# ymxlzgy/commonscenes

Hardware: AMD Instinct MI355X
Metric: DDIM denoise steps/sec (32 objects, 16^3 latent) (higher is better)
Workload: dtype f32 (operands as fp16 hi+lo pairs, fp32 accumulate)

## Files before the change

commonscenes_amd/csrc/cs_epilogue.h:

```cpp
#pragma once
#include "cs_common.h"

typedef unsigned cs_u32x4 __attribute__((ext_vector_type(4)));

template <class D, class M>
__device__ __forceinline__ f32x4 cs_epi_terms4(const D& d, f32x4 v, M m, int n) {
  if (d.bias) v += *reinterpret_cast<const f32x4*>(d.bias + n);
  if (d.scale) v = v * *reinterpret_cast<const f32x4*>(d.scale + n) + *reinterpret_cast<const f32x4*>(d.shift + n);
  if (d.rowvec) v += *reinterpret_cast<const f32x4*>(d.rowvec + (int64_t)(m / d.rv_rows) * d.ldrv + n);
  if (d.act != CS_ACT_NONE) {
#pragma unroll
    for (int e = 0; e < 4; ++e) v[e] = cs_act(v[e], d.act);
  }
  if (d.res) v += *reinterpret_cast<const f32x4*>(d.res + (int64_t)m * d.ldr + n);
  return v;
}
template <class D>
__device__ __forceinline__ float cs_epi_terms1(const D& d, float v, float bias, float scale, float shift, int m, int n) {
  v += bias;
  if (d.scale) v = v * scale + shift;
  if (d.rowvec) v += d.rowvec[(int64_t)(m / d.rv_rows) * d.ldrv + n];
  v = cs_act(v, d.act);
  if (d.res) v += d.res[(int64_t)m * d.ldr + n];
  return v;
}

__device__ __forceinline__ f32x4 cs_geglu4(f32x4 x, const f32x4& g) {
#pragma unroll
  for (int e = 0; e < 4; ++e) x[e] = x[e] * cs_gelu(g[e]);
  return x;
}

__device__ __forceinline__ cs_u32x4 cs_pair16(const f32x4& v, float out_scale, bool odd, float& oamax) {
  typedef _Float16 h4 __attribute__((ext_vector_type(4)));
  typedef unsigned u32x2 __attribute__((ext_vector_type(2)));
  h4 hi, lo;
#pragma unroll
  for (int e = 0; e < 4; ++e) {
    const float o = v[e] * out_scale;
    oamax = fmaxf(oamax, fabsf(o));
    hi[e] = (_Float16)o;
    lo[e] = (_Float16)(o - (float)hi[e]);
  }
  const u32x2 H = __builtin_bit_cast(u32x2, hi), L = __builtin_bit_cast(u32x2, lo);
  const u32x2 send = odd ? H : L;
  u32x2 recv;
  recv[0] = (unsigned)__builtin_amdgcn_update_dpp(0, (int)send[0], 0xB1, 0xF, 0xF, true);
  recv[1] = (unsigned)__builtin_amdgcn_update_dpp(0, (int)send[1], 0xB1, 0xF, 0xF, true);
  cs_u32x4 r;
  r[0] = odd ? recv[0] : H[0];
  r[1] = odd ? recv[1] : H[1];
  r[2] = odd ? L[0] : recv[0];
  r[3] = odd ? L[1] : recv[1];
  return r;
}
__device__ __forceinline__ int cs_pair_off(int col) { return (col >> 4) * 64 + ((col & 8) ? 32 : 0) + ((col & 4) ? 16 : 0); }
template <class D>
__device__ __forceinline__ void cs_pair_flag(const D& d, bool opair, float oamax) {
  if (opair && d.status && oamax >= 65504.f) atomicOr(d.status, CS_STATUS_F16X3_OVERFLOW);
}

__device__ __forceinline__ void cs_colsum_lanes16(double (*sc)[64], const double (&x)[4], int rl, int cl, double (&tot)[4]) {
  __syncthreads();
#pragma unroll
  for (int e = 0; e < 4; ++e) sc[rl][cl * 4 + e] = x[e];
  __syncthreads();
  if (rl == 0) {
#pragma unroll
    for (int e = 0; e < 4; ++e) {
      double t = 0.0;
      for (int r2 = 0; r2 < 16; ++r2) t += sc[r2][cl * 4 + e];
      tot[e] = t;
    }
  }
}
template <class D>
__device__ __forceinline__ void cs_colsum_staged(const D& d, const float* col, int ld, int rows, int tile, int n) {
  double ts = 0.0, tq = 0.0;
  for (int r2 = 0; r2 < rows; ++r2) {
    const double x = (double)col[r2 * ld];
    ts += x;
    tq += x * x;
  }
  double* o = d.gn_part + ((int64_t)tile * d.gn_ld + n) * 2;
  o[0] = ts;
  o[1] = tq;
}
```

commonscenes_amd/csrc/cs_gemm_f16x3.hip:

```cpp
#include <cstdlib>
#include <cstring>
#include "cs_f16x3.h"
#include "cs_epilogue.h"
#include <type_traits>
#include <utility>

namespace {

using cs16::h8;
using cs16::split8;
using cs16::wait_vmcnt;
using cs16::BKH;
using cs16::A_SCALE_DEFAULT;
using cs16::OOB;
constexpr int MAX_TAPS = 27;
#ifndef CS_ABLATE
#define CS_ABLATE 0
#endif

struct CsClsBatch {
  const void* w[8];
  const void* w_lo[8];
  float acc_scale[8];
  int n;
};

template <int NT, int BM, int BN>
__device__ __forceinline__ void fused_splitk_reduce(const CsFuseK& f, const float* __restrict__ ws, unsigned char* smem, int M,
                                                    int cout, int m0, int n0, int splits, int otile, int tid) {
  typedef unsigned u32x4 __attribute__((ext_vector_type(4)));
  typedef unsigned u32x2 __attribute__((ext_vector_type(2)));
  typedef _Float16 h4 __attribute__((ext_vector_type(4)));
  int32_t* const arrive = f.sync + 2 * otile;
  asm volatile("s_waitcnt vmcnt(0)" ::: "memory");
  __syncthreads();
  int* const tick = reinterpret_cast<int*>(smem);
  if (tid == 0) *tick = __hip_atomic_fetch_add(arrive, 1, __ATOMIC_RELAXED, __HIP_MEMORY_SCOPE_AGENT);
  __syncthreads();
  const int R = f.reducers;
  const int split = *tick - (splits - R);
  if (split < 0) return;
  if (tid == 0) {
    int spins = 0;
    while (__hip_atomic_load(arrive, __ATOMIC_RELAXED, __HIP_MEMORY_SCOPE_AGENT) < splits) {
      __builtin_amdgcn_s_sleep(4);
      if (++spins > (1 << 23)) {
        if (f.status) atomicOr(f.status, CS_STATUS_SPLITK_TIMEOUT);
        break;
      }
    }
  }
  __syncthreads();
  constexpr int C4 = BN / 4;
  constexpr int UNITS = 16 * C4;
  static_assert(UNITS % 2 == 0 && BN <= NT && 16 * BN * 4 <= 32768, "fused split-K reduce geometry");
  float* const lv = reinterpret_cast<float*>(smem);
  const __amdgpu_buffer_rsrc_t wrs = __builtin_amdgcn_make_buffer_rsrc(
      (void*)ws, 0, (unsigned)((int64_t)splits * M * cout * 4), 0x00020000);
  const bool gstat = f.gn_part != nullptr, opair = f.out_format == 2;
  const int rows_per = BM / R;
  float oamax = 0.f;
  for (int blk = 0; blk < rows_per / 16; ++blk) {
    const int r0 = split * rows_per + 16 * blk;
    if (m0 + r0 >= M) break;
    for (int u0 = 0; u0 < UNITS; u0 += NT) {
      const int u = u0 + tid;
      const int lrow = u / C4, c4 = u - lrow * C4;
      const int m = m0 + r0 + lrow, n = n0 + 4 * c4;
      const bool ok = u < UNITS && m < M && n < cout;
      f32x4 v = {0.f, 0.f, 0.f, 0.f};
      if (ok) {
        const unsigned off0 = (unsigned)(((int64_t)m * cout + n) * 4);
        const unsigned sstride = (unsigned)((int64_t)M * cout * 4);
        v = __builtin_bit_cast(f32x4, __builtin_amdgcn_raw_buffer_load_b128(wrs, off0, 0, 16));
        for (int s = 1; s < splits; s += 8) {
          f32x4 t[8];
#pragma unroll
          for (int q = 0; q < 8; ++q)
            if (s + q < splits)
              t[q] = __builtin_bit_cast(f32x4, __builtin_amdgcn_raw_buffer_load_b128(wrs, off0 + (unsigned)(s + q) * sstride, 0, 16));
#pragma unroll
          for (int q = 0; q < 8; ++q)
            if (s + q < splits) v += t[q];
        }
        v = cs_epi_terms4(f, v, m, n);
      }
      if (gstat && u < UNITS) *reinterpret_cast<f32x4*>(lv + lrow * BN + 4 * c4) = v;
      if (opair) {
        h4 hi, lo;
#pragma unroll
        for (int e = 0; e < 4; ++e) {
          const float o = v[e] * f.out_scale;
          oamax = fmaxf(oamax, fabsf(o));
          hi[e] = (_Float16)o;
          lo[e] = (_Float16)(o - (float)hi[e]);
        }
        const u32x2 H = __builtin_bit_cast(u32x2, hi), L = __builtin_bit_cast(u32x2, lo);
        const bool odd = tid & 1;
        const u32x2 send = odd ? H : L;
        u32x2 recv;
        recv[0] = (unsigned)__builtin_amdgcn_update_dpp(0, (int)send[0], 0xB1, 0xF, 0xF, true);
        recv[1] = (unsigned)__builtin_amdgcn_update_dpp(0, (int)send[1], 0xB1, 0xF, 0xF, true);
        u32x4 r;
        r[0] = odd ? recv[0] : H[0];
        r[1] = odd ? recv[1] : H[1];
        r[2] = odd ? L[0] : recv[0];
        r[3] = odd ? L[1] : recv[1];
        if (ok) {
          char* row = reinterpret_cast<char*>(f.out + (int64_t)m * f.ldo);
          *reinterpret_cast<u32x4*>(row + (n >> 4) * 64 + ((n & 8) ? 32 : 0) + ((n & 4) ? 16 : 0)) = r;
        }
      } else if (ok) {
        *reinterpret_cast<f32x4*>(f.out + (int64_t)m * f.ldo + n) = v;
      }
    }
    if (gstat) {
      __syncthreads();
      if (tid < BN && n0 + tid < cout) {
        double ts = 0.0, tq = 0.0;
#pragma unroll
        for (int r2 = 0; r2 < 16; ++r2) {
          const double d = (double)lv[r2 * BN + tid];
          ts += d;
          tq += d * d;
        }
        double* o = f.gn_part + ((int64_t)((m0 + r0) / 16) * f.gn_ld + n0 + tid) * 2;
        o[0] = ts;
        o[1] = tq;
      }
      __syncthreads();
    }
  }
  cs_pair_flag(f, opair, oamax);
  __syncthreads();
  if (tid == 0) {
    const int d = __hip_atomic_fetch_add(arrive + 1, 1, __ATOMIC_RELAXED, __HIP_MEMORY_SCOPE_AGENT);
    if (d == R - 1) {
      __hip_atomic_store(arrive, 0, __ATOMIC_RELAXED, __HIP_MEMORY_SCOPE_AGENT);
      __hip_atomic_store(arrive + 1, 0, __ATOMIC_RELAXED, __HIP_MEMORY_SCOPE_AGENT);
    }
  }
}

template <class F, int... I>
__device__ __forceinline__ void static_steps(std::integer_sequence<int, I...>, F&& f) {
  (f(std::integral_constant<int, I>{}), ...);
}

template <int WMB, int WNB, int WAVES_M, int WAVES_N, bool PRE, int SLAB = 0, bool PAIR = false, int TPK = 9, bool PW = false>
__global__ __launch_bounds__(64 * WAVES_M * WAVES_N, 2) void conv_gemm_f16x3_kernel(const CsConvGemm p, int M, int tiles_n,
                                                              int taps_hw, int kw_, int kg_per_tap,
                                                              long long x_bytes, unsigned w_bytes, int vec_epilogue,
                                                              int splits, int omap_f, int omap_p_in, const CsClsBatch cb,
                                                              const CsFuseK fz, int u_base, int u_count) {
  constexpr int BM = 32 * WMB * WAVES_M;
  constexpr int BN = 32 * WNB * WAVES_N;
  constexpr int NW = WAVES_M * WAVES_N;
  constexpr int NT = 64 * NW;
  static_assert(!SLAB || (WMB <= 2 && WAVES_N == 1), "slab path: one or two row blocks per wave");
  static_assert(!PAIR || (!PRE && SLAB == 0), "interleaved operand pairs: per-tap gather path only");
  static_assert(TPK == 9 || ((TPK == 4 || TPK == 3) && SLAB != 0), "taps per kd: 3x3 or (slab path only) 2x2 / 3x1");
  static_assert(!PW || SLAB == 0, "pointwise GEMMs take the gather path (there is one tap)");
  constexpr int KW_ = TPK == 9 ? 3 : TPK == 4 ? 2 : 1;
  constexpr int KH_ = TPK / KW_;
  constexpr int SLAB_ROWS = BM + (KH_ - 1) * SLAB + (KW_ - 1);
  constexpr int SLAB_IMG_WI = (SLAB_ROWS + 31) / 32;
  constexpr int SLAB_WI = PRE ? 2 * SLAB_IMG_WI : (SLAB_ROWS + 15) / 16;
  constexpr int SLAB_IMG = SLAB_IMG_WI * 1024;
  constexpr int SLAB_BYTES = SLAB ? SLAB_WI * 1024 : 0;
  constexpr int RING0 = 2 * SLAB_BYTES;
  constexpr int A_BYTES = SLAB ? 0 : BM * 64;
  constexpr int B_BYTES = 2 * BN * 16;
  constexpr int STAGE = A_BYTES + 2 * B_BYTES;
#ifdef CS_RING3
  constexpr int NSTAGE = 3;
#else
#ifdef CS_PW_RING3
  constexpr int NSTAGE = (BM == 64 && BN == 64) ? 6 : (TPK == 4 ? 4 : 3);
#else
#ifndef CS_RING64
#define CS_RING64 6
#endif
  constexpr int NSTAGE = (BM == 64 && BN == 64) ? CS_RING64 : ((TPK == 4 || (PW && BM == 256 && BN == 224)) ? 4 : 3);
#endif
#endif
  constexpr int PF = NSTAGE - 1;
  constexpr int DUMP = RING0 + NSTAGE * STAGE;
  constexpr int ROWBASE = DUMP + 1024;
  constexpr int DELTA = ROWBASE + (SLAB ? 0 : BM * 4);
  constexpr int ROWMIN = DELTA + (SLAB ? 0 : MAX_TAPS * BM * 2);
  constexpr int EP_KU = (4 * (32 * WNB / 4) + 63) / 64;
  constexpr int EPI_NEED = NW * (16 * 32 * WNB) + NW * 2 * EP_KU * 1024 + 2048;
  constexpr int OTAB = ((ROWMIN + 16 > EPI_NEED) ? ROWMIN + 16 : EPI_NEED);
  constexpr int LDS_BYTES = OTAB + (TPK == 4 ? BM * 4 : 0);
  constexpr short INVALID = (short)0x8000;
  constexpr int A_WI = BM / 16;
  constexpr int B_WI = BN / 32;
  constexpr int A_PW = SLAB ? 0 : A_WI / NW;
  constexpr int A_PWN = A_PW > 0 ? A_PW : 1;
  constexpr int B_PW = (2 * B_WI + NW - 1) / NW;
  constexpr int D = A_PW + B_PW;
  static_assert(A_WI % NW == 0, "A tile must split evenly over the waves");
  static_assert(D <= 7, "vmcnt immediates");
  __shared__ __attribute__((aligned(16))) unsigned char smem[LDS_BYTES];

  const int tid = threadIdx.x;
  const int lane = tid & 63;
  const int wave = __builtin_amdgcn_readfirstlane(tid >> 6);
  const int l31 = lane & 31;
  const int half = lane >> 5;
  const int wm0 = (wave / WAVES_N) * (32 * WMB);
  const int wn0 = (wave % WAVES_N) * (32 * WNB);

  int tile;
  {
    const int nblk = gridDim.x, b = blockIdx.x;
    const int q = nblk >> 3, r = nblk & 7, xcd = b & 7, within = b >> 3;
    tile = (xcd < r ? xcd * (q + 1) : r * (q + 1) + (xcd - r) * q) + within;
  }
  const void* w_hi_ = p.w;
  const void* w_lo_ = p.w_lo;
  float acc_scale_ = p.acc_scale;
  int pad_d = p.pd, pad_h = p.ph, pad_w = p.pw, omap_p = omap_p_in;
  int cls_id = 0;
  if constexpr (TPK == 4) {
    if (cb.n > 1) {
      const int per_cls = ((M + BM - 1) / BM) * tiles_n * splits;
      const int cls = tile / per_cls;
      cls_id = cls;
      tile -= cls * per_cls;
      w_hi_ = cb.w[cls];
      w_lo_ = cb.w_lo[cls];
      acc_scale_ = cb.acc_scale[cls];
      const int nw = 1 + (omap_f & 1), nh = 1 + ((omap_f >> 1) & 1);
      const int qw = cls % nw, qh = (cls / nw) % nh, qd = cls / (nw * nh);
      pad_d = (omap_f & 4) ? 1 - qd : 1;
      pad_h = (omap_f & 2) ? 1 - qh : 1;
      pad_w = (omap_f & 1) ? 1 - qw : 1;
      omap_p = (qd << 2) | (qh << 1) | qw;
    }
  }
  int split, tn, tm;
  if (TPK == 3 && u_count > 0) {
    const int R = ((M + BM - 1) / BM) / (omap_p_in > 1 ? omap_p_in : 1);
    const int r = tile % R;
    tile /= R;
    split = tile % splits;
    const int u = u_base + tile / splits;
    tn = u % tiles_n;
    tm = (u / tiles_n) * R + r;
  } else if (SLAB != 0 && splits > 1) {
    const int tiles_m = (M + BM - 1) / BM;
    tm = tile % tiles_m;
    tile /= tiles_m;
    split = tile % splits;
    tn = tile / splits;
  } else {
    split = tile % splits;
    tile /= splits;
    tn = tile % tiles_n;
    tm = tile / tiles_n;
  }
  const int m0 = tm * BM;
  const int n0 = tn * BN;
  if constexpr (TPK == 3) {
    if (omap_p_in > 1) {
      const int tiles_m = (M + BM - 1) / BM;
      const int q = tm / (tiles_m / omap_p_in);
      w_hi_ = reinterpret_cast<const char*>(p.w) + (size_t)q * w_bytes;
      w_lo_ = reinterpret_cast<const char*>(p.w_lo) + (size_t)q * w_bytes;
    }
  }

  const __amdgpu_buffer_rsrc_t hrs = __builtin_amdgcn_make_buffer_rsrc((void*)w_hi_, 0, w_bytes, 0x00020000);
  const __amdgpu_buffer_rsrc_t lrs = __builtin_amdgcn_make_buffer_rsrc((void*)w_lo_, 0, w_bytes, 0x00020000);

  const int ntaps = p.kd * taps_hw;
  int* rowbase = reinterpret_cast<int*>(smem + ROWBASE);
  int* rowmin = reinterpret_cast<int*>(smem + ROWMIN);
  short* delta = reinterpret_cast<short*>(smem + DELTA);
  if constexpr (!SLAB && !PW) {
  if (tid == 0) *rowmin = 0x7fffffff;
  __syncthreads();
  {
    const int vdin = p.din << p.ud, vhin = p.hin << p.uh, vwin = p.win << p.uw;
    constexpr int TPR = NT / BM >= 1 ? NT / BM : 1;
    for (int row = tid / TPR; row < BM; row += NT / TPR) {
      const int sub = tid % TPR;
      const int m = m0 + row;
      int mm = m < M ? m : 0;
      const int ow = mm % p.wout;
      mm /= p.wout;
      const int oh = mm % p.hout;
      mm /= p.hout;
      const int od = mm % p.dout;
      const int n = mm / p.dout;
      const int cd = min(max(od * p.sd - pad_d, 0), vdin - 1) >> p.ud;
      const int ch = min(max(oh * p.sh - pad_h, 0), vhin - 1) >> p.uh;
      const int cw = min(max(ow * p.sw - pad_w, 0), vwin - 1) >> p.uw;
      const int base = ((n * p.din + cd) * p.hin + ch) * p.win + cw;
      if (sub == 0) {
        rowbase[row] = base;
        if (m < M) atomicMin(rowmin, base);
      }
      const int vd0 = od * p.sd - pad_d, vh0 = oh * p.sh - pad_h, vw0 = ow * p.sw - pad_w;
      int t = 0;
      for (int kd_ = 0; kd_ < p.kd; ++kd_)
        for (int kh_ = 0; kh_ < p.kh; ++kh_)
          for (int kwi = 0; kwi < kw_; ++kwi, ++t) {
            if (t % TPR != sub) continue;
            short dl = INVALID;
            const int vd = vd0 + kd_, vh = vh0 + kh_, vw = vw0 + kwi;
            if (m < M && (unsigned)vd < (unsigned)vdin && (unsigned)vh < (unsigned)vhin &&
                (unsigned)vw < (unsigned)vwin) {
              const int r = ((n * p.din + (vd >> p.ud)) * p.hin + (vh >> p.uh)) * p.win + (vw >> p.uw);
              dl = (short)(r - base);
            }
            delta[t * BM + row] = dl;
          }
    }
  }
  __syncthreads();
  }

  const int row_lo = SLAB ? max(0, m0 - pad_d * p.hin * p.win - pad_h * p.win - pad_w)
                     : PW ? m0 : __builtin_amdgcn_readfirstlane(*rowmin);
  const long long x_skip = (long long)row_lo * p.lda * (PRE ? 2 : 4);
  const long long x_left = x_bytes - x_skip;
  const unsigned x_win = x_left > 0xFFE00000LL ? 0xFFE00000u : (unsigned)x_left;
  const __amdgpu_buffer_rsrc_t xrs =
      __builtin_amdgcn_make_buffer_rsrc((void*)((const char*)p.x + x_skip), 0, x_win, 0x00020000);
  const __amdgpu_buffer_rsrc_t xlrs = __builtin_amdgcn_make_buffer_rsrc(
      (void*)((const char*)(PRE ? p.x_lo : (const void*)p.x) + x_skip), 0, x_win, 0x00020000);

  float a_scale = p.a_scale;
  if constexpr (!PRE && !PAIR) {
    if (p.a_bound) {
      const float m = *p.a_bound;
      int ex = 0;
      float s2 = 1.0995116e12f;
      if (m > 0.f && m < 3.0e38f) {
        (void)frexpf(65000.0f / m, &ex);
        s2 = ldexpf(1.0f, min(max(ex - 1, -8), 40));
      }
      acc_scale_ *= a_scale / s2;
      a_scale = s2;
    }
  }
  const int chunks_per_tap = kg_per_tap >> 1;
  const int nk_all = ntaps * chunks_per_tap;
  constexpr int KGRAN = SLAB ? TPK : 1;
  const int per_split = ((nk_all / KGRAN + splits - 1) / splits) * KGRAN;
  const int k_first = split * per_split;
#if CS_ABLATE & 2048
  const int nk = 0;
#else
  const int nk = max(0, min(nk_all, k_first + per_split) - k_first);
#endif

  int a_rowbase[A_PWN];
  unsigned a_piece[A_PWN];
  int a_rowidx[A_PWN];
#pragma unroll
  for (int i = 0; i < A_PW; ++i) {
    const int w = wave * A_PW + i;
    if constexpr (PRE) {
      const int within = w % (A_WI / 2);
      const int row = 32 * within + (lane >> 1);
      a_rowidx[i] = row;
      if constexpr (PW) a_rowbase[i] = (m0 + row < M) ? row : -1;
      else a_rowbase[i] = rowbase[row] - row_lo;
      a_piece[i] = (unsigned)(((lane & 1) ^ ((row >> 3) & 1)) * 8);
    } else {
      const int row = 16 * w + (lane >> 2);
      a_rowidx[i] = row;
      if constexpr (PW) a_rowbase[i] = (m0 + row < M) ? row : -1;
      else a_rowbase[i] = rowbase[row] - row_lo;
      a_piece[i] = (unsigned)(((lane & 3) ^ ((row >> 2) & 3)) * 4);
    }
  }
  unsigned b_off[B_PW];
#pragma unroll
  for (int i = 0; i < B_PW; ++i) {
    const int v = wave * B_PW + i;
    const int img = v / B_WI;
    const int u = (v - img * B_WI) * 64 + lane;
    const int kg = u / BN;
    const int n = u - kg * BN;
    b_off[i] = (v < 2 * B_WI && n0 + n < p.cout) ? (unsigned)((kg * p.cout + n0 + n) * 16) : OOB;
  }

  auto issue_dma = [&](int tap, int cc, int stage) {
    unsigned char* st = smem + RING0 + stage * STAGE;
    const bool skip_a = ((CS_ABLATE & 128) && tap % 3 != 0) || ((CS_ABLATE & 256) && tap % 9 != 0);
#pragma unroll
    for (int i = 0; i < A_PW; ++i) {
      if (skip_a) break;
      const int c = cc * BKH + (int)a_piece[i];
      constexpr unsigned ESZ = PRE ? 2u : 4u;
      unsigned off;
      if constexpr (PW) {
        off = (a_rowbase[i] >= 0 && c < p.cin) ? (unsigned)a_rowbase[i] * ((unsigned)p.lda * ESZ) + (unsigned)c * ESZ : OOB;
      } else {
        const short dl = delta[tap * BM + a_rowidx[i]];
        off = (dl != INVALID && c < p.cin)
                  ? (unsigned)(a_rowbase[i] + (int)dl) * ((unsigned)p.lda * ESZ) + (unsigned)c * ESZ
                  : OOB;
      }
      if (CS_ABLATE & 2) off = OOB;
      if ((CS_ABLATE & 64) && off != OOB) off &= 0x3FF0u;
      const int w = wave * A_PW + i;
      if constexpr (PRE) {
        if (w >= A_WI / 2)
          __builtin_amdgcn_raw_ptr_buffer_load_lds(xlrs, st + w * 1024, 16, off, 0, 0, 0);
        else
          __builtin_amdgcn_raw_ptr_buffer_load_lds(xrs, st + w * 1024, 16, off, 0, 0, 0);
      } else {
        __builtin_amdgcn_raw_ptr_buffer_load_lds(xrs, st + w * 1024, 16, off, 0, 0, 0);
      }
    }
    const unsigned kbase = (unsigned)((tap * kg_per_tap + cc * 2) * p.cout) * 16u;
#pragma unroll
    for (int i = 0; i < B_PW; ++i) {
      const int v = wave * B_PW + i;
      const int img = v / B_WI;
      unsigned off = (b_off[i] == OOB || cc >= chunks_per_tap) ? OOB : b_off[i] + kbase;
      if (CS_ABLATE & 2) off = OOB;
      if ((CS_ABLATE & 64) && off != OOB) off &= 0x3FF0u;
      unsigned char* dst = (v < 2 * B_WI) ? st + A_BYTES + img * B_BYTES + (v - img * B_WI) * 1024 : smem + DUMP;
      if (img == 1)
        __builtin_amdgcn_raw_ptr_buffer_load_lds(lrs, dst, 16, off, 0, 0, 0);
      else
        __builtin_amdgcn_raw_ptr_buffer_load_lds(hrs, dst, 16, off, 0, 0, 0);
    }
  };

  f32x16 acc[WMB][WNB];
#pragma unroll
  for (int i = 0; i < WMB; ++i)
#pragma unroll
    for (int j = 0; j < WNB; ++j)
#pragma unroll
      for (int r = 0; r < 16; ++r) acc[i][j][r] = 0.f;

  int dtap = k_first % ntaps, dcc = k_first / ntaps;
  auto advance = [&]() {
    if (++dtap == ntaps) {
      dtap = 0;
      ++dcc;
    }
  };
#pragma unroll
  for (int q = 0; q < PF; ++q) {
    issue_dma(dtap, dcc, q);
    advance();
  }

  int a_frag[WMB][2];
#pragma unroll
  for (int i = 0; i < WMB; ++i) {
    const int row = wm0 + 32 * i + l31;
    if constexpr (PRE) {
      a_frag[i][0] = row * 32 + ((half ^ ((row >> 3) & 1)) * 16);
      a_frag[i][1] = a_frag[i][0] + BM * 32;
    } else {
      const int s = (row >> 2) & 3;
      a_frag[i][0] = row * 64 + (((2 * half) ^ s) * 16);
      a_frag[i][1] = row * 64 + (((2 * half + 1) ^ s) * 16);
    }
  }
  const int b_frag = A_BYTES + (half * BN + wn0 + l31) * 16;

  float amax = 0.f;
  auto load_a = [&](int st, h8 (&hi)[WMB], h8 (&lo)[WMB]) {
    const unsigned char* s = smem + RING0 + st * STAGE;
#pragma unroll
    for (int i = 0; i < WMB; ++i) {
      if constexpr (PRE) {
        hi[i] = *reinterpret_cast<const h8*>(s + a_frag[i][0]);
        lo[i] = *reinterpret_cast<const h8*>(s + a_frag[i][1]);
      } else {
        const f32x4 x0 = *reinterpret_cast<const f32x4*>(s + a_frag[i][0]);
        const f32x4 x1 = *reinterpret_cast<const f32x4*>(s + a_frag[i][1]);
#if CS_ABLATE & 512
        hi[i] = __builtin_bit_cast(h8, x0);
        lo[i] = __builtin_bit_cast(h8, x1);
#else
        if constexpr (PAIR) {
          hi[i] = __builtin_bit_cast(h8, x0);
          lo[i] = __builtin_bit_cast(h8, x1);
        } else {
          split8(x0, x1, a_scale, hi[i], lo[i], amax);
        }
#endif
      }
    }
  };
  constexpr int SLAB_PW = (SLAB_WI + NW - 1) / NW;
  const int s_w = p.win, s_hw = p.hin * p.win;
  const int s_rows = p.nb * p.din * s_hw;
  const int s_need = BM + (KH_ - 1) * s_w + (KW_ - 1);
  unsigned vmask[WMB];
  int sl_row[SLAB_PW];
  unsigned sl_piece[SLAB_PW];
  int sl_a0[WMB][TPK];
  if constexpr (SLAB != 0) {
#pragma unroll
    for (int i = 0; i < WMB; ++i) {
      const int rowl = wm0 + 32 * i + l31;
#pragma unroll
      for (int t9 = 0; t9 < TPK; ++t9) {
        const int prow = rowl + (t9 / KW_) * s_w + t9 % KW_;
        if constexpr (PRE)
          sl_a0[i][t9] = prow * 32 + (((half ^ (prow >> 3)) & 1) << 4);
        else
          sl_a0[i][t9] = prow * 64 + ((((2 * half) ^ (prow >> 2)) & 3) << 4);
      }
      vmask[i] = 0;
      const int m = m0 + rowl;
      if (m < M) {
        int mm = m;
        const int ow = mm % p.win;
        mm /= p.win;
        const int oh = mm % p.hin;
        mm /= p.hin;
        const int od = mm % p.din;
#pragma unroll
        for (int t = 0; t < 3 * TPK; ++t) {
          const int kd_ = t / TPK, kh_ = (t % TPK) / KW_, kwi = t % KW_;
          if ((unsigned)(od + kd_ - pad_d) < (unsigned)p.din && (unsigned)(oh + kh_ - pad_h) < (unsigned)p.hin &&
              (unsigned)(ow + kwi - pad_w) < (unsigned)p.win)
            vmask[i] |= 1u << t;
        }
      }
    }
    if constexpr (PRE) {
      if (tid < 4) reinterpret_cast<int*>(smem + ROWMIN)[tid] = 0;
      __syncthreads();
    }
#pragma unroll
    for (int i = 0; i < SLAB_PW; ++i) {
      if constexpr (PRE) {
        const int j = 32 * ((wave + NW * i) % SLAB_IMG_WI) + (lane >> 1);
        sl_row[i] = j;
        sl_piece[i] = (unsigned)(((lane & 1) ^ ((j >> 3) & 1)) * 8);
        continue;
      }
      const int j = 16 * (wave + NW * i) + (lane >> 2);
      sl_row[i] = j;
      sl_piece[i] = (unsigned)(((lane & 3) ^ ((j >> 2) & 3)) * 4);
    }
  }
  const int KD = p.kd;
  auto issue_slab = [&](int sc) {
    const int cc = sc / KD, kd_ = sc - KD * cc;
    const int src0 = m0 + (kd_ - pad_d) * s_hw - pad_h * s_w - pad_w;
    unsigned char* dst = smem + (sc & 1) * SLAB_BYTES;
#pragma unroll
    for (int i = 0; i < SLAB_PW; ++i) {
      const int q = wave + NW * i;
      const int src = src0 + sl_row[i];
      const int c = cc * BKH + (int)sl_piece[i];
      constexpr unsigned ESZ = PRE ? 2u : 4u;
      const unsigned off = (q < SLAB_WI && sl_row[i] < s_need && src >= 0 && src < s_rows && c < p.cin && cc < chunks_per_tap)
                               ? (unsigned)(src - row_lo) * ((unsigned)p.lda * ESZ) + (unsigned)c * ESZ
                               : OOB;
      unsigned char* d2 = q < SLAB_WI ? dst + q * 1024 : smem + DUMP;
      if (PRE && q >= SLAB_IMG_WI)
        __builtin_amdgcn_raw_ptr_buffer_load_lds(xlrs, d2, 16, off, 0, 0, 0);
      else
        __builtin_amdgcn_raw_ptr_buffer_load_lds(xrs, d2, 16, off, 0, 0, 0);
    }
  };
  auto load_a_slab = [&](auto t9_c, int i, int buf, unsigned m9, h8& hi, h8& lo) {
    constexpr int t9 = decltype(t9_c)::value;
    if constexpr (PRE) {
      const bool ok = (m9 >> t9) & 1u;
      const int a = buf * SLAB_BYTES + sl_a0[i][t9];
      hi = *reinterpret_cast<const h8*>(smem + (ok ? a : ROWMIN));
      lo = *reinterpret_cast<const h8*>(smem + (ok ? a + SLAB_IMG : ROWMIN));
      return;
    }
    const unsigned char* sb = smem + buf * SLAB_BYTES;
    const f32x4 x0 = *reinterpret_cast<const f32x4*>(sb + sl_a0[i][t9]);
    const f32x4 x1 = *reinterpret_cast<const f32x4*>(sb + (sl_a0[i][t9] ^ 16));
#if CS_ABLATE & 512
    hi = __builtin_bit_cast(h8, x0);
    lo = __builtin_bit_cast(h8, x1);
    (void)m9;
#else
    cs16::split8_masked(x0, x1, ((m9 >> t9) & 1u) ? a_scale : 0.f, hi, lo, amax);
#endif
  };

  h8 ah[WMB], al[WMB];
  if constexpr (SLAB != 0) {
    const int sc0 = k_first / TPK;
    issue_slab(sc0);
    wait_vmcnt<0>();
    __builtin_amdgcn_s_barrier();
#pragma unroll
    for (int i = 0; i < WMB; ++i)
      load_a_slab(std::integral_constant<int, 0>{}, i, sc0 & 1, (vmask[i] >> (TPK * (sc0 % KD))) & ((1u << TPK) - 1u), ah[i],
                  al[i]);
  } else {
  wait_vmcnt<(PF - 1) * D>();
  __builtin_amdgcn_s_barrier();
  load_a(0, ah, al);
  }

  auto step = [&](auto stage_c) {
    constexpr int stage = decltype(stage_c)::value;
    constexpr int nstage = (stage + 1) % NSTAGE;
    constexpr int dstage = (stage + PF) % NSTAGE;
    if (!(CS_ABLATE & 4)) wait_vmcnt<(PF - 2) * D + B_PW>();
    if (!(CS_ABLATE & 8)) __builtin_amdgcn_s_barrier();
    const unsigned char* s = smem + RING0 + stage * STAGE;
    h8 ah2[WMB], al2[WMB];
#if CS_ABLATE & 16
    __builtin_amdgcn_s_setprio(1);
#endif
#pragma unroll
    for (int j = 0; j < WNB; ++j) {
      const h8 bh = *reinterpret_cast<const h8*>(s + b_frag + j * 512);
      const h8 bl = *reinterpret_cast<const h8*>(s + b_frag + B_BYTES + j * 512);
#pragma unroll
      for (int i = 0; i < WMB; ++i) {
        acc[i][j] = __builtin_amdgcn_mfma_f32_32x32x16_f16(al[i], bh, acc[i][j], 0, 0, 0);
        acc[i][j] = __builtin_amdgcn_mfma_f32_32x32x16_f16(ah[i], bl, acc[i][j], 0, 0, 0);
        acc[i][j] = __builtin_amdgcn_mfma_f32_32x32x16_f16(ah[i], bh, acc[i][j], 0, 0, 0);
      }
      if (j == 0) {
        if (!(CS_ABLATE & 1)) issue_dma(dtap, dcc, dstage);
        advance();
        load_a(nstage, ah2, al2);
      }
    }
#if CS_ABLATE & 16
    __builtin_amdgcn_s_setprio(0);
#endif
#pragma unroll
    for (int i = 0; i < WMB; ++i) {
      ah[i] = ah2[i];
      al[i] = al2[i];
    }
  };
  auto sstep = [&](auto stage_c, auto t9_c, int sc, const unsigned (&m9_this)[WMB], const unsigned (&m9_next)[WMB]) {
    constexpr int stage = decltype(stage_c)::value;
    constexpr int t9 = decltype(t9_c)::value;
    constexpr int dstage = (stage + PF) % NSTAGE;
    if (!(CS_ABLATE & 4)) wait_vmcnt<((t9 >= 1 && t9 <= PF - 1) ? SLAB_PW : 0) + (PF - 1) * B_PW>();
    if (!(CS_ABLATE & 8)) __builtin_amdgcn_s_barrier();
    const unsigned char* s = smem + RING0 + stage * STAGE;
    h8 ah2[WMB], al2[WMB];
    h8 bh, bl;
#pragma unroll
    for (int j = 0; j < WNB; ++j) {
      if (!(((CS_ABLATE & 4096) && (j & 1)) || ((CS_ABLATE & 8192) && j > 0))) {
        bh = *reinterpret_cast<const h8*>(s + b_frag + j * 512);
        bl = *reinterpret_cast<const h8*>(s + b_frag + B_BYTES + j * 512);
      }
#pragma unroll
      for (int i = 0; i < WMB; ++i) {
        acc[i][j] = __builtin_amdgcn_mfma_f32_32x32x16_f16(al[i], bh, acc[i][j], 0, 0, 0);
        acc[i][j] = __builtin_amdgcn_mfma_f32_32x32x16_f16(ah[i], bl, acc[i][j], 0, 0, 0);
        acc[i][j] = __builtin_amdgcn_mfma_f32_32x32x16_f16(ah[i], bh, acc[i][j], 0, 0, 0);
      }
      if (j == 0) {
        if constexpr (t9 == 0) issue_slab(sc + 1);
        issue_dma(dtap, dcc, dstage);
        advance();
#pragma unroll
        for (int i = 0; i < WMB; ++i) {
          if constexpr (t9 == TPK - 1)
            load_a_slab(std::integral_constant<int, 0>{}, i, (sc + 1) & 1, m9_next[i], ah2[i], al2[i]);
          else
            load_a_slab(std::integral_constant<int, t9 + 1>{}, i, sc & 1, m9_this[i], ah2[i], al2[i]);
        }
      }
    }
#pragma unroll
    for (int i = 0; i < WMB; ++i) {
      ah[i] = ah2[i];
      al[i] = al2[i];
    }
  };
  if constexpr (SLAB != 0) {
    static_assert(((TPK == 9 || TPK == 3) && NSTAGE == 3) || (TPK == 4 && NSTAGE == 4), "a chunk's ring stage is its tap index mod NSTAGE");
    const int sc_first = k_first / TPK, sc_end = sc_first + nk / TPK;
    int kdc = sc_first % KD;
    constexpr unsigned TMASK = (1u << TPK) - 1u;
    for (int sc = sc_first; sc < sc_end; ++sc) {
      const int kdn = kdc == KD - 1 ? 0 : kdc + 1;
      unsigned m9[WMB], m9n[WMB];
#pragma unroll
      for (int i = 0; i < WMB; ++i) {
        m9[i] = (vmask[i] >> (TPK * kdc)) & TMASK;
        m9n[i] = (vmask[i] >> (TPK * kdn)) & TMASK;
      }
      if constexpr (TPK == 9) {
        sstep(std::integral_constant<int, 0>{}, std::integral_constant<int, 0>{}, sc, m9, m9n);
        sstep(std::integral_constant<int, 1>{}, std::integral_constant<int, 1>{}, sc, m9, m9n);
        sstep(std::integral_constant<int, 2>{}, std::integral_constant<int, 2>{}, sc, m9, m9n);
        sstep(std::integral_constant<int, 0>{}, std::integral_constant<int, 3>{}, sc, m9, m9n);
        sstep(std::integral_constant<int, 1>{}, std::integral_constant<int, 4>{}, sc, m9, m9n);
        sstep(std::integral_constant<int, 2>{}, std::integral_constant<int, 5>{}, sc, m9, m9n);
        sstep(std::integral_constant<int, 0>{}, std::integral_constant<int, 6>{}, sc, m9, m9n);
        sstep(std::integral_constant<int, 1>{}, std::integral_constant<int, 7>{}, sc, m9, m9n);
        sstep(std::integral_constant<int, 2>{}, std::integral_constant<int, 8>{}, sc, m9, m9n);
      } else if constexpr (TPK == 3) {
        sstep(std::integral_constant<int, 0>{}, std::integral_constant<int, 0>{}, sc, m9, m9n);
        sstep(std::integral_constant<int, 1>{}, std::integral_constant<int, 1>{}, sc, m9, m9n);
        sstep(std::integral_constant<int, 2>{}, std::integral_constant<int, 2>{}, sc, m9, m9n);
      } else {
        sstep(std::integral_constant<int, 0>{}, std::integral_constant<int, 0>{}, sc, m9, m9n);
        sstep(std::integral_constant<int, 1>{}, std::integral_constant<int, 1>{}, sc, m9, m9n);
        sstep(std::integral_constant<int, 2>{}, std::integral_constant<int, 2>{}, sc, m9, m9n);
        sstep(std::integral_constant<int, 3>{}, std::integral_constant<int, 3>{}, sc, m9, m9n);
      }
      kdc = kdn;
    }
  } else
  for (int kc = 0; kc < nk; kc += NSTAGE) {
    step(std::integral_constant<int, 0>{});
    static_steps(std::make_integer_sequence<int, NSTAGE - 1>{}, [&](auto s1) {
      constexpr int st = decltype(s1)::value + 1;
      if (kc + st < nk) step(std::integral_constant<int, st>{});
    });
  }
  wait_vmcnt<0>();
  if constexpr (!PRE && !PAIR) {
    if (p.status && amax >= 65504.f) atomicOr(p.status, CS_STATUS_F16X3_OVERFLOW);
  }

#if CS_ABLATE & 1024
  {
    float sum = 0.f;
#pragma unroll
    for (int i = 0; i < WMB; ++i)
#pragma unroll
      for (int j = 0; j < WNB; ++j)
#pragma unroll
        for (int r = 0; r < 16; ++r) sum += acc[i][j][r];
    if (M == -12345) p.out[tid] = sum;
    return;
  }
#endif
  float* const outp = p.out + ((int64_t)cls_id * splits + split) * M * p.ldo;
  const bool omap = (TPK == 4) && (omap_f & 7) != 0 && !(omap_f & 8);
  int* const otab = reinterpret_cast<int*>(smem + OTAB);
  long long ob = m0, Mo = M;
  int ospan = BM;
  if constexpr (TPK == 4) {
    if (omap) {
      const int fd = 1 + ((omap_f >> 2) & 1), fh = 1 + ((omap_f >> 1) & 1), fw = 1 + (omap_f & 1);
      const int qd = (omap_p >> 2) & 1, qh = (omap_p >> 1) & 1, qw = omap_p & 1;
      auto orow = [&](int m) -> long long {
        const int w = m % p.win;
        int t = m / p.win;
        const int h = t % p.hin;
        t /= p.hin;
        const int d = t % p.din;
        const int n = t / p.din;
        return (((long long)n * (p.din * fd) + d * fd + qd) * (p.hin * fh) + h * fh + qh) * (p.win * fw) + w * fw + qw;
      };
      ob = orow(m0);
      Mo = (long long)M * (fd * fh * fw);
      const int mlast = min(m0 + BM, M) - 1;
      ospan = (int)(orow(mlast) - ob) + 1;
      for (int r = tid; r < BM; r += NT) otab[r] = (m0 + r < M) ? (int)(orow(m0 + r) - ob) : 0;
      __syncthreads();
    }
  }
  auto orel = [&](int row) -> int { return omap ? otab[row] : row; };
  constexpr int WCOLS = 32 * WNB;
  constexpr int PASS_R = (NW * 16 * WCOLS * 4 <= DUMP) ? 8 : 4;
  constexpr int EPI_ROWS = 2 * PASS_R;
  constexpr int EPI_BYTES = EPI_ROWS * WCOLS * 4;
  static_assert(NW * EPI_BYTES <= DUMP, "epilogue staging must fit in the ring");
  {
    typedef cs_u32x4 u32x4;
    constexpr int QR = 2;
    constexpr int NQ = 16 / QR;
    constexpr int UPR = WCOLS / 4;
    constexpr int UN = 2 * QR * UPR;
    constexpr int KU = (UN + 63) / 64;
    constexpr int EPB = 2 * QR * WCOLS * 4;
    constexpr int RSLAB = KU * 1024;
    constexpr int RES0 = NW * EPB;
    constexpr int VEC0 = RES0 + NW * 2 * RSLAB;
    constexpr int BNV = (BN + 63) / 64;
    static_assert(VEC0 + 2048 <= LDS_BYTES && BN <= 256 && BNV <= NW, "pipelined epilogue must fit in the kernel's LDS");
    const int m_last = min(m0 + BM, M) - 1;
    const bool geglu = p.act == CS_ACT_GEGLU;
    const bool has_res = p.res != nullptr;
#ifndef CS_PIPED_PLAIN
#define CS_PIPED_PLAIN 1
#endif
    const bool piped = !(CS_ABLATE & 32) && vec_epilogue && (p.res || p.bias || p.rowvec || CS_PIPED_PLAIN) && !p.scale && splits == 1 &&
                       (!geglu || n0 + BN <= p.cout) && (!p.rowvec || (m0 / p.rv_rows == m_last / p.rv_rows)) &&
                       (long long)ospan * p.ldo * 4 < 0x7FF00000LL && (!p.res || (long long)BM * p.ldr * 4 < 0x7FF00000LL);
    const bool gstat = p.gn_part != nullptr;
    const bool opair = p.out_format == 2;
    if ((gstat || opair) && !piped && tid == 0 && p.status) atomicOr(p.status, CS_STATUS_INTERNAL);
    if (piped) {
      __syncthreads();
      float* const ep = reinterpret_cast<float*>(smem + wave * EPB);
      typedef float f32x2 __attribute__((ext_vector_type(2)));
      f32x2 gs[KU][2], gq[KU][2];
#pragma unroll
      for (int k = 0; k < KU; ++k)
#pragma unroll
        for (int e = 0; e < 2; ++e) gs[k][e] = gq[k][e] = f32x2{0.f, 0.f};
      float oamax = 0.f;
      float* const rs = reinterpret_cast<float*>(smem + RES0 + wave * 2 * RSLAB);
      float* const vb = reinterpret_cast<float*>(smem + VEC0);
      float* const vr = vb + 256;
      const long long o_skip = ob * p.ldo * 4, r_skip = (long long)m0 * p.ldr * 4;
      const long long o_left = ((Mo - 1) * p.ldo + p.cout) * 4 - o_skip;
      const long long r_left = has_res ? ((long long)(M - 1) * p.ldr + p.cout) * 4 - r_skip : 0;
      const long long o_cols = geglu ? p.cout / 2 : p.cout;
      const long long o_left2 = ((Mo - 1) * p.ldo + o_cols) * 4 - o_skip;
      (void)o_left;
      const __amdgpu_buffer_rsrc_t ors = __builtin_amdgcn_make_buffer_rsrc(
          (void*)((char*)p.out + o_skip), 0, o_left2 > 0x7FF00000LL ? 0x7FF00000u : (unsigned)o_left2, 0x00020000);
      const __amdgpu_buffer_rsrc_t rrs = __builtin_amdgcn_make_buffer_rsrc(
          (void*)(has_res ? (const char*)p.res + r_skip : (const char*)p.out), 0,
          r_left > 0x7FF00000LL ? 0x7FF00000u : (r_left > 0 ? (unsigned)r_left : 0u), 0x00020000);
      if (wave < BNV) {
        const unsigned col = (unsigned)(64 * wave + lane);
        const unsigned off = col < (unsigned)BN ? (unsigned)(n0 + (int)col) * 4u : OOB;
        if (p.bias) {
          const __amdgpu_buffer_rsrc_t brs = __builtin_amdgcn_make_buffer_rsrc((void*)p.bias, 0, (unsigned)p.cout * 4u, 0x00020000);
          __builtin_amdgcn_raw_ptr_buffer_load_lds(brs, vb + 64 * wave, 4, off, 0, 0, 0);
        }
        if (p.rowvec) {
          const __amdgpu_buffer_rsrc_t vrs = __builtin_amdgcn_make_buffer_rsrc(
              (void*)(p.rowvec + (int64_t)(m0 / p.rv_rows) * p.ldrv), 0, (unsigned)p.cout * 4u, 0x00020000);
          __builtin_amdgcn_raw_ptr_buffer_load_lds(vrs, vr + 64 * wave, 4, off, 0, 0, 0);
        }
      }
      auto pass_row = [&](int i, int q, int lrow) {
        return wm0 + 32 * i + 2 * (q & 1) + 8 * (q >> 1) + (lrow & 1) + 4 * (lrow >> 1);
      };
      auto fetch_res = [&](int pass) {
        const int i = pass / NQ, q = pass - i * NQ;
#pragma unroll
        for (int k = 0; k < KU; ++k) {
          const int u = lane + 64 * k;
          const int lrow = u / UPR, c4 = u - lrow * UPR;
          const int row = pass_row(i, q, lrow & 3);
          const unsigned off = (u < UN && m0 + row < M) ? (unsigned)(row * p.ldr + n0 + wn0 + 4 * c4) * 4u : OOB;
          __builtin_amdgcn_raw_ptr_buffer_load_lds(rrs, rs + (pass & 1) * (RSLAB / 4) + 256 * k, 16, off, 0, 0, 0);
        }
      };
      if (has_res) {
        fetch_res(0);
        wait_vmcnt<KU>();
      } else {
        wait_vmcnt<0>();
      }
      __syncthreads();
      constexpr int NPASS = WMB * NQ;
      auto do_pass = [&](auto i_c, auto q_c) {
        constexpr int i = decltype(i_c)::value, q = decltype(q_c)::value, pass = i * NQ + q;
        if (has_res) {
          if constexpr (pass + 1 < NPASS) fetch_res(pass + 1);
          wait_vmcnt<(pass > 0 ? KU : 0) + (pass + 1 < NPASS ? KU : 0)>();
        }
#pragma unroll
        for (int j = 0; j < WNB; ++j)
#pragma unroll
          for (int rr = 0; rr < QR; ++rr) ep[(rr + QR * half) * WCOLS + 32 * j + l31] = acc[i][j][QR * q + rr] * acc_scale_;
        if (geglu) {
          constexpr int HC = WCOLS / 2, UPG = HC / 4 > 0 ? HC / 4 : 1, UNG = 2 * QR * UPG, KG = (UNG + 63) / 64;
#pragma unroll
          for (int k = 0; k < KG; ++k) {
            const int u = lane + 64 * k;
            const int lrow = u / UPG, c4 = u - lrow * UPG;
            const int row = pass_row(i, q, lrow & 3);
            f32x4 xv = {0.f, 0.f, 0.f, 0.f};
            unsigned off = OOB;
            const bool ok = u < UNG && m0 + row < M;
            if (ok) {
              xv = *reinterpret_cast<const f32x4*>(ep + lrow * WCOLS + 4 * c4);
              f32x4 gv = *reinterpret_cast<const f32x4*>(ep + lrow * WCOLS + HC + 4 * c4);
              if (p.bias) {
                xv += *reinterpret_cast<const f32x4*>(vb + wn0 + 4 * c4);
                gv += *reinterpret_cast<const f32x4*>(vb + wn0 + HC + 4 * c4);
              }
              xv = (CS_ABLATE & 32768) ? xv * gv : cs_geglu4(xv, gv);
              off = (unsigned)(orel(row) * p.ldo + (n0 + wn0) / 2 + 4 * c4) * 4u;
            }
            if (opair) {
              const u32x4 pk = cs_pair16(xv, p.out_scale, lane & 1, oamax);
              if (ok) off = (unsigned)(orel(row) * p.ldo) * 4u + (unsigned)cs_pair_off((n0 + wn0) / 2 + 4 * c4);
              if (CS_ABLATE & 16384) off = OOB;
              __builtin_amdgcn_raw_buffer_store_b128(pk, ors, off, 0, 0);
            } else {
              __builtin_amdgcn_raw_buffer_store_b128(__builtin_bit_cast(u32x4, xv), ors, off, 0, 0);
            }
          }
          return;
        }
#pragma unroll
        for (int k = 0; k < KU; ++k) {
          const int u = lane + 64 * k;
          const int lrow = u / UPR, c4 = u - lrow * UPR;
          const int row = pass_row(i, q, lrow & 3);
          f32x4 v = {0.f, 0.f, 0.f, 0.f};
          unsigned off = OOB;
          const bool ok = u < UN && m0 + row < M && n0 + wn0 + 4 * c4 < p.cout;
          if (ok) {
            v = *reinterpret_cast<const f32x4*>(ep + lrow * WCOLS + 4 * c4);
            if (p.bias) v += *reinterpret_cast<const f32x4*>(vb + wn0 + 4 * c4);
            if (p.rowvec) v += *reinterpret_cast<const f32x4*>(vr + wn0 + 4 * c4);
            if (p.act != CS_ACT_NONE) {
#pragma unroll
              for (int e = 0; e < 4; ++e) v[e] = cs_act(v[e], p.act);
            }
            if (has_res) v += *reinterpret_cast<const f32x4*>(rs + (pass & 1) * (RSLAB / 4) + 4 * u);
            off = (unsigned)(orel(row) * p.ldo + n0 + wn0 + 4 * c4) * 4u;
            if (gstat) {
              const f32x2 lo2 = {v[0], v[1]}, hi2 = {v[2], v[3]};
              gs[k][0] += lo2;
              gs[k][1] += hi2;
              gq[k][0] = __builtin_elementwise_fma(lo2, lo2, gq[k][0]);
              gq[k][1] = __builtin_elementwise_fma(hi2, hi2, gq[k][1]);
            }
          }
          if (CS_ABLATE & 16384) off = OOB;
          if (opair) {
            const u32x4 pk = cs_pair16(v, p.out_scale, lane & 1, oamax);
            if (ok && !(CS_ABLATE & 16384)) off = (unsigned)(orel(row) * p.ldo) * 4u + (unsigned)cs_pair_off(n0 + wn0 + 4 * c4);
            __builtin_amdgcn_raw_buffer_store_b128(pk, ors, off, 0, 0);
          } else {
            __builtin_amdgcn_raw_buffer_store_b128(__builtin_bit_cast(u32x4, v), ors, off, 0, 0);
          }
        }
      };
      auto all_q = [&](auto i_c) {
        do_pass(i_c, std::integral_constant<int, 0>{});
        do_pass(i_c, std::integral_constant<int, 1>{});
        do_pass(i_c, std::integral_constant<int, 2>{});
        do_pass(i_c, std::integral_constant<int, 3>{});
        do_pass(i_c, std::integral_constant<int, 4>{});
        do_pass(i_c, std::integral_constant<int, 5>{});
        do_pass(i_c, std::integral_constant<int, 6>{});
        do_pass(i_c, std::integral_constant<int, 7>{});
      };
      all_q(std::integral_constant<int, 0>{});
      if constexpr (WMB > 1) all_q(std::integral_constant<int, 1>{});
      static_assert(WMB <= 2 && NQ == 8, "pass enumeration");
      cs_pair_flag(p, opair, oamax);
      if (gstat) {
        static_assert(NW * 4 * WCOLS * 8 <= LDS_BYTES && BN <= NT, "statistics scratch must fit the kernel's LDS");
        f32x2* const sc = reinterpret_cast<f32x2*>(smem);
// ... 364 lines not shown
```

Measured before the change: 15.76.

## Transpose MFMA operands in pointwise GEMMs for row-contiguous direct-store epilogue

For pointwise GEMM instantiations, the MFMA operand order is swapped so each lane's accumulators hold contiguous output columns of one row. A new epilogue then writes 128-bit stores straight from registers, reading bias and row-vector values that were DMA'd into LDS at kernel start. Paired fp16 hi/lo output uses a permlane32 swap instead of a DPP exchange. This is meant to bypass the LDS staging in the pipelined epilogue. Paths it does not cover, such as group-norm statistics, first untranspose the accumulators through LDS scratch, which adds LDS traffic there.

```diff
diff --git a/commonscenes_amd/csrc/cs_epilogue.h b/commonscenes_amd/csrc/cs_epilogue.h
--- a/commonscenes_amd/csrc/cs_epilogue.h
+++ b/commonscenes_amd/csrc/cs_epilogue.h
@@ -54,6 +54,27 @@
   r[3] = odd ? L[1] : recv[1];
   return r;
 }
+__device__ __forceinline__ cs_u32x4 cs_pair16_half32(const f32x4& v, float out_scale, float& oamax) {
+  typedef _Float16 h4 __attribute__((ext_vector_type(4)));
+  typedef unsigned u32x2 __attribute__((ext_vector_type(2)));
+  h4 hi, lo;
+#pragma unroll
+  for (int e = 0; e < 4; ++e) {
+    const float o = v[e] * out_scale;
+    oamax = fmaxf(oamax, fabsf(o));
+    hi[e] = (_Float16)o;
+    lo[e] = (_Float16)(o - (float)hi[e]);
+  }
+  const u32x2 H = __builtin_bit_cast(u32x2, hi), L = __builtin_bit_cast(u32x2, lo);
+  const auto s0 = __builtin_amdgcn_permlane32_swap(H[0], L[0], false, false);
+  const auto s1 = __builtin_amdgcn_permlane32_swap(H[1], L[1], false, false);
+  cs_u32x4 r;
+  r[0] = s0[0];
+  r[1] = s1[0];
+  r[2] = s0[1];
+  r[3] = s1[1];
+  return r;
+}
 __device__ __forceinline__ int cs_pair_off(int col) { return (col >> 4) * 64 + ((col & 8) ? 32 : 0) + ((col & 4) ? 16 : 0); }
 template <class D>
 __device__ __forceinline__ void cs_pair_flag(const D& d, bool opair, float oamax) {
diff --git a/commonscenes_amd/csrc/cs_gemm_f16x3.hip b/commonscenes_amd/csrc/cs_gemm_f16x3.hip
--- a/commonscenes_amd/csrc/cs_gemm_f16x3.hip
+++ b/commonscenes_amd/csrc/cs_gemm_f16x3.hip
@@ -157,6 +157,7 @@
   constexpr int BN = 32 * WNB * WAVES_N;
   constexpr int NW = WAVES_M * WAVES_N;
   constexpr int NT = 64 * NW;
+  constexpr bool TR = PW;
   static_assert(!SLAB || (WMB <= 2 && WAVES_N == 1), "slab path: one or two row blocks per wave");
   static_assert(!PAIR || (!PRE && SLAB == 0), "interleaved operand pairs: per-tap gather path only");
   static_assert(TPK == 9 || ((TPK == 4 || TPK == 3) && SLAB != 0), "taps per kd: 3x3 or (slab path only) 2x2 / 3x1");
@@ -435,6 +436,25 @@
     }
   };
 
+  constexpr int TRV = ROWBASE;
+  if constexpr (TR) {
+    static_assert(TRV + 2048 <= LDS_BYTES && BN <= 256 && (BN + 63) / 64 <= NW, "bias / row-vector rows beyond the ring");
+    if (wave < (BN + 63) / 64) {
+      const unsigned col = (unsigned)(64 * wave + lane);
+      const unsigned off = col < (unsigned)BN ? (unsigned)(n0 + (int)col) * 4u : OOB;
+      float* const tv = reinterpret_cast<float*>(smem + TRV);
+      if (p.bias) {
+        const __amdgpu_buffer_rsrc_t brs = __builtin_amdgcn_make_buffer_rsrc((void*)p.bias, 0, (unsigned)p.cout * 4u, 0x00020000);
+        __builtin_amdgcn_raw_ptr_buffer_load_lds(brs, tv + 64 * wave, 4, off, 0, 0, 0);
+      }
+      if (p.rowvec) {
+        const __amdgpu_buffer_rsrc_t vrs = __builtin_amdgcn_make_buffer_rsrc(
+            (void*)(p.rowvec + (int64_t)(m0 / p.rv_rows) * p.ldrv), 0, (unsigned)p.cout * 4u, 0x00020000);
+        __builtin_amdgcn_raw_ptr_buffer_load_lds(vrs, tv + 256 + 64 * wave, 4, off, 0, 0, 0);
+      }
+    }
+  }
+
   f32x16 acc[WMB][WNB];
 #pragma unroll
   for (int i = 0; i < WMB; ++i)
@@ -626,9 +646,15 @@
       const h8 bl = *reinterpret_cast<const h8*>(s + b_frag + B_BYTES + j * 512);
 #pragma unroll
       for (int i = 0; i < WMB; ++i) {
-        acc[i][j] = __builtin_amdgcn_mfma_f32_32x32x16_f16(al[i], bh, acc[i][j], 0, 0, 0);
-        acc[i][j] = __builtin_amdgcn_mfma_f32_32x32x16_f16(ah[i], bl, acc[i][j], 0, 0, 0);
-        acc[i][j] = __builtin_amdgcn_mfma_f32_32x32x16_f16(ah[i], bh, acc[i][j], 0, 0, 0);
+        if constexpr (TR) {
+          acc[i][j] = __builtin_amdgcn_mfma_f32_32x32x16_f16(bh, al[i], acc[i][j], 0, 0, 0);
+          acc[i][j] = __builtin_amdgcn_mfma_f32_32x32x16_f16(bl, ah[i], acc[i][j], 0, 0, 0);
+          acc[i][j] = __builtin_amdgcn_mfma_f32_32x32x16_f16(bh, ah[i], acc[i][j], 0, 0, 0);
+        } else {
+          acc[i][j] = __builtin_amdgcn_mfma_f32_32x32x16_f16(al[i], bh, acc[i][j], 0, 0, 0);
+          acc[i][j] = __builtin_amdgcn_mfma_f32_32x32x16_f16(ah[i], bl, acc[i][j], 0, 0, 0);
+          acc[i][j] = __builtin_amdgcn_mfma_f32_32x32x16_f16(ah[i], bh, acc[i][j], 0, 0, 0);
+        }
       }
       if (j == 0) {
         if (!(CS_ABLATE & 1)) issue_dma(dtap, dcc, dstage);
@@ -803,6 +829,138 @@
     const bool gstat = p.gn_part != nullptr;
     const bool opair = p.out_format == 2;
     if ((gstat || opair) && !piped && tid == 0 && p.status) atomicOr(p.status, CS_STATUS_INTERNAL);
+    if constexpr (TR) {
+      if (piped && !gstat) {
+        typedef cs_u32x4 u32x4;
+        constexpr int NG = 4 * WNB;
+        constexpr int GB = (WMB * NG <= 16) ? NG : NG / 2;
+        static_assert(NG % GB == 0 && WMB * GB <= 16, "residual batches");
+        const long long o_skip = (long long)m0 * p.ldo * 4, r_skip = (long long)m0 * p.ldr * 4;
+        const long long o_cols = geglu ? p.cout / 2 : p.cout;
+        const long long o_left = ((long long)(M - 1) * p.ldo + o_cols) * 4 - o_skip;
+        const long long r_left = has_res ? ((long long)(M - 1) * p.ldr + p.cout) * 4 - r_skip : 0;
+        const __amdgpu_buffer_rsrc_t ors = __builtin_amdgcn_make_buffer_rsrc(
+            (void*)((char*)p.out + o_skip), 0, o_left > 0x7FF00000LL ? 0x7FF00000u : (unsigned)o_left, 0x00020000);
+        const __amdgpu_buffer_rsrc_t rrs = __builtin_amdgcn_make_buffer_rsrc(
+            (void*)(has_res ? (const char*)p.res + r_skip : (const char*)p.out), 0,
+            r_left > 0x7FF00000LL ? 0x7FF00000u : (r_left > 0 ? (unsigned)r_left : 0u), 0x00020000);
+        const float* const tvb = reinterpret_cast<const float*>(smem + TRV) + wn0 + 4 * half;
+        const float* const tvr = tvb + 256;
+        const int cl = n0 + wn0 + 4 * half;
+        bool rok[WMB];
+        unsigned orow[WMB], rrow[WMB];
+#pragma unroll
+        for (int i = 0; i < WMB; ++i) {
+          const int row = wm0 + 32 * i + l31;
+          rok[i] = m0 + row < M;
+          orow[i] = (unsigned)(row * p.ldo) * 4u;
+          rrow[i] = (unsigned)(row * p.ldr) * 4u;
+        }
+        float oamax = 0.f;
+        if (geglu) {
+          constexpr int HG = NG / 2;
+          const int co = (n0 + wn0) / 2 + 4 * half;
+#pragma unroll
+          for (int t = 0; t < HG; ++t) {
+            f32x4 bx = {0.f, 0.f, 0.f, 0.f}, bg = bx;
+            if (p.bias) {
+              bx = *reinterpret_cast<const f32x4*>(tvb + 8 * t);
+              bg = *reinterpret_cast<const f32x4*>(tvb + 8 * (t + HG));
+            }
+#pragma unroll
+            for (int i = 0; i < WMB; ++i) {
+              f32x4 xv, gv;
+#pragma unroll
+              for (int e = 0; e < 4; ++e) {
+                xv[e] = acc[i][t / 4][4 * (t % 4) + e] * acc_scale_;
+                gv[e] = acc[i][(t + HG) / 4][4 * ((t + HG) % 4) + e] * acc_scale_;
+              }
+              if (p.bias) {
+                xv += bx;
+                gv += bg;
+              }
+              xv = (CS_ABLATE & 32768) ? xv * gv : cs_geglu4(xv, gv);
+              const bool ok = rok[i];
+              if (opair) {
+                if (!ok) xv = f32x4{0.f, 0.f, 0.f, 0.f};
+                const u32x4 pk = cs_pair16_half32(xv, p.out_scale, oamax);
+                unsigned off = ok ? orow[i] + (unsigned)cs_pair_off(co + 8 * t) : OOB;
+                if (CS_ABLATE & 16384) off = OOB;
+                __builtin_amdgcn_raw_buffer_store_b128(pk, ors, off, 0, 0);
+              } else {
+                unsigned off = ok ? orow[i] + (unsigned)(co + 8 * t) * 4u : OOB;
+                if (CS_ABLATE & 16384) off = OOB;
+                __builtin_amdgcn_raw_buffer_store_b128(__builtin_bit_cast(u32x4, xv), ors, off, 0, 0);
+              }
+            }
+          }
+        } else {
+#pragma unroll
+          for (int t0 = 0; t0 < NG; t0 += GB) {
+            f32x4 rv[WMB][GB];
+            if (has_res) {
+#pragma unroll
+              for (int i = 0; i < WMB; ++i)
+#pragma unroll
+                for (int tt = 0; tt < GB; ++tt) {
+                  const int n = cl + 8 * (t0 + tt);
+                  const unsigned off = (rok[i] && n < p.cout) ? rrow[i] + (unsigned)n * 4u : OOB;
+                  rv[i][tt] = __builtin_bit_cast(f32x4, __builtin_amdgcn_raw_buffer_load_b128(rrs, off, 0, 0));
+                }
+            }
+#pragma unroll
+            for (int tt = 0; tt < GB; ++tt) {
+              const int t = t0 + tt;
+              const int n = cl + 8 * t;
+              f32x4 bv = {0.f, 0.f, 0.f, 0.f}, vv = bv;
+              if (p.bias) bv = *reinterpret_cast<const f32x4*>(tvb + 8 * t);
+              if (p.rowvec) vv = *reinterpret_cast<const f32x4*>(tvr + 8 * t);
+#pragma unroll
+              for (int i = 0; i < WMB; ++i) {
+                f32x4 v;
+#pragma unroll
+                for (int e = 0; e < 4; ++e) v[e] = acc[i][t / 4][4 * (t % 4) + e] * acc_scale_;
+                if (p.bias) v += bv;
+                if (p.rowvec) v += vv;
+                if (p.act != CS_ACT_NONE) {
+#pragma unroll
+                  for (int e = 0; e < 4; ++e) v[e] = cs_act(v[e], p.act);
+                }
+                if (has_res) v += rv[i][tt];
+                const bool ok = rok[i] && n < p.cout;
+                if (opair) {
+                  if (!ok) v = f32x4{0.f, 0.f, 0.f, 0.f};
+                  const u32x4 pk = cs_pair16_half32(v, p.out_scale, oamax);
+                  unsigned off = ok ? orow[i] + (unsigned)cs_pair_off(n) : OOB;
+                  if (CS_ABLATE & 16384) off = OOB;
+                  __builtin_amdgcn_raw_buffer_store_b128(pk, ors, off, 0, 0);
+                } else {
+                  unsigned off = ok ? orow[i] + (unsigned)n * 4u : OOB;
+                  if (CS_ABLATE & 16384) off = OOB;
+                  __builtin_amdgcn_raw_buffer_store_b128(__builtin_bit_cast(u32x4, v), ors, off, 0, 0);
+                }
+              }
+            }
+          }
+        }
+        cs_pair_flag(p, opair, oamax);
+        return;
+      }
+      {
+        static_assert(NW * 32 * 33 * 4 <= DUMP, "untranspose scratch must fit in the ring");
+        __syncthreads();
+        float* const tb = reinterpret_cast<float*>(smem) + wave * (32 * 33);
+#pragma unroll
+        for (int i = 0; i < WMB; ++i)
+#pragma unroll
+          for (int j = 0; j < WNB; ++j) {
+#pragma unroll
+            for (int r = 0; r < 16; ++r) tb[l31 * 33 + 8 * (r >> 2) + 4 * half + (r & 3)] = acc[i][j][r];
+#pragma unroll
+            for (int r = 0; r < 16; ++r) acc[i][j][r] = tb[(8 * (r >> 2) + 4 * half + (r & 3)) * 33 + l31];
+          }
+      }
+    }
     if (piped) {
       __syncthreads();
       float* const ep = reinterpret_cast<float*>(smem + wave * EPB);
```

After: 15.96 (median of 6 runs). 1.3% higher.
